# HannesStark/3DInfomax

Hardware: AMD Instinct MI355X
Metric: molecules/sec pretraining step (PNA+Net3D, QM9-50k); PNA-agg HBM GB/s vs peak (higher is better)
Workload: dtype f32

## Files before the change

3dinfomax_amd/csrc/wgrad.hip:

```cpp
#include "common.h"

#include <algorithm>
#include <cstdlib>
#include <cstring>

namespace i3d {
namespace {

typedef float floatx4 __attribute__((ext_vector_type(4)));
typedef int intx4 __attribute__((ext_vector_type(4)));
typedef short shortx4 __attribute__((ext_vector_type(4)));
typedef __bf16 bf16x4_t __attribute__((ext_vector_type(4)));

constexpr int PREC_F32 = 0, PREC_BF16 = 1, PREC_BF16X3 = 2;

__device__ __forceinline__ void split4(const float v[4], shortx4& hi, shortx4& lo, const bool want_lo) {
    const bf16x4_t h = {(__bf16)v[0], (__bf16)v[1], (__bf16)v[2], (__bf16)v[3]};
    hi = __builtin_bit_cast(shortx4, h);
    if (want_lo) {
        const bf16x4_t l = {(__bf16)(v[0] - (float)h[0]), (__bf16)(v[1] - (float)h[1]), (__bf16)(v[2] - (float)h[2]),
                            (__bf16)(v[3] - (float)h[3])};
        lo = __builtin_bit_cast(shortx4, l);
    }
}
typedef __attribute__((address_space(3))) void* lds_ptr_t;

constexpr int WG_T = 13;
constexpr int WG_LD = 208;
constexpr int WG_LDP = 256;
constexpr int WG_BK = 16;
constexpr int wg_nst(int prec) { return prec == 0 ? 2 : 3; }
constexpr int WG_UNIT_FLOATS = WG_T * WG_T * 256;
constexpr int WG_MAX_PROBLEMS = 40;
constexpr int WG_MAX_SLICE = 1024;
constexpr int WG_MAX_OUTPUTS = 8;

struct WgProb {
    const float* A;
    const float* B;
    const int* rows;
    unsigned a_bytes, b_bytes;
    int lda, ldb;
    int M, N;
    int mcw, ncw;
    int m_chunks, n_chunks;
    int k_begin, k_end, k_per_slice;
    int unit_begin;
};

struct WgArgs {
    float* slab;
    unsigned long long* stamps;
    int n_problems, n_units;
    WgProb p[WG_MAX_PROBLEMS];
};

__device__ __forceinline__ int xcd_unit(int total) {
    const int id = blockIdx.x;
    const int q = total / 8, r = total % 8, xcd = id % 8;
    return xcd * q + min(xcd, r) + id / 8;
}

#ifdef WG_TIMING
#define WG_STAMP(i) do { if (threadIdx.x == 0) stamps[i] = __builtin_readcyclecounter(); } while (0)
#else
#define WG_STAMP(i) do { } while (0)
#endif

template <int MT, bool NFULL, int PREC>
__device__ __forceinline__ void wgrad_unit(const WgProb& p, const int slice, const int mc, const int nc, float* __restrict__ out,
                                           float* __restrict__ smem, int* __restrict__ kidx, unsigned long long* stamps) {
    WG_STAMP(0);
    constexpr int NQ = MT == WG_T ? 4 : (MT + 3) / 4;
    const int lane = threadIdx.x & 63, wave = __builtin_amdgcn_readfirstlane(threadIdx.x >> 6);
    const int l15 = lane & 15, lk = lane >> 4;
    const int k0 = p.k_begin + slice * p.k_per_slice;
// ... 17 lines not shown
    float* const Bs = smem + NST * WG_BK * WG_LDP;
    const unsigned as_base = (unsigned)(unsigned long long)(lds_ptr_t)As, bs_base = (unsigned)(unsigned long long)(lds_ptr_t)Bs;
    __syncthreads();

    int rnext[4];
    auto read_rows = [&](int t) {
#pragma unroll
        for (int i = 0; i < 4; ++i) rnext[i] = kidx[min(t * WG_BK + wave + 4 * i, klen - 1)];
    };
    auto issue_piece = [&](int t, int buf, int i) {
        const int kr = wave + 4 * i;
        const int kl = t * WG_BK + kr;
        const bool live = kl < klen && rnext[i] >= 0;
        const unsigned oa = (live && a_ok) ? (unsigned)rnext[i] * lda4 + col : a_rec;
        const unsigned ob = (live && b_ok) ? (unsigned)rnext[i] * ldb4 + col : b_rec;
        const unsigned la = as_base + (unsigned)((buf * WG_BK + kr) * WG_LDP) * 4u;
        const unsigned lb = bs_base + (unsigned)((buf * WG_BK + kr) * WG_LDP) * 4u;
        unsigned keep;
        asm volatile("s_mov_b32 %0, m0\n\ts_mov_b32 m0, %1\n\ts_nop 0\n\tbuffer_load_dwordx4 %2, %3, 0 offen lds\n\t"
                     "s_mov_b32 m0, %4\n\ts_nop 0\n\tbuffer_load_dwordx4 %5, %6, 0 offen lds\n\ts_mov_b32 m0, %0"
                     : "=&s"(keep)
                     : "s"(__builtin_amdgcn_readfirstlane(la)), "v"(oa), "s"(da), "s"(__builtin_amdgcn_readfirstlane(lb)), "v"(ob), "s"(db)
                     : "memory");
    };

    floatx4 acc[3][MT], accx[NQ];
#pragma unroll
    for (int j = 0; j < 3; ++j)
#pragma unroll
        for (int i = 0; i < MT; ++i) acc[j][i] = floatx4{0.f, 0.f, 0.f, 0.f};
#pragma unroll
    for (int q = 0; q < NQ; ++q) accx[q] = floatx4{0.f, 0.f, 0.f, 0.f};

    const int nkt = (klen + WG_BK - 1) / WG_BK;
#pragma unroll
    for (int t0 = 0; t0 < NST - 1; ++t0) {
        read_rows(t0);
#pragma unroll
        for (int i = 0; i < 4; ++i) issue_piece(t0, t0, i);
    }
    if constexpr (NST == 2) asm volatile("s_waitcnt vmcnt(0)" ::: "memory");
    else asm volatile("s_waitcnt vmcnt(8)" ::: "memory");
    __syncthreads();
    WG_STAMP(1);
    const bool extra = ntl == WG_T;
    const int b = lk & 1;
    const int even_off = lk * WG_LDP + l15 + 16 * b, odd_off = lk * WG_LDP + l15 - 16 * b;
    const int own_off = pw ? odd_off : even_off;
    for (int t = 0; t < nkt; ++t) {
        const int cur = t % NST, nxt = (t + NST - 1) % NST;
        read_rows(t + NST - 1);
        const float* as = As + cur * WG_BK * WG_LDP;
        const float* bs = Bs + cur * WG_BK * WG_LDP;
        if constexpr (PREC != PREC_F32) {
            constexpr bool X3 = PREC == PREC_BF16X3;
            auto frag = [&](const float* base, int off, shortx4& hi, shortx4& lo) {
                float v[4];
#pragma unroll
                for (int kk = 0; kk < 4; ++kk) v[kk] = base[kk * 4 * WG_LDP + off];
                split4(v, hi, lo, X3);
            };
            auto fma3 = [&](floatx4& c, const shortx4& bh, const shortx4& bl, const shortx4& ah, const shortx4& al) {
                if constexpr (X3) {
                    c = __builtin_amdgcn_mfma_f32_16x16x16bf16_1k(bl, ah, c, 0, 0, 0);
                    c = __builtin_amdgcn_mfma_f32_16x16x16bf16_1k(bh, al, c, 0, 0, 0);
                }
                c = __builtin_amdgcn_mfma_f32_16x16x16bf16_1k(bh, ah, c, 0, 0, 0);
            };
            shortx4 bh[3], bl[3], bxh, bxl;
#pragma unroll
            for (int j = 0; j < 3; ++j) frag(bs, own_off + (wave + 4 * j) * 16, bh[j], bl[j]);
            frag(bs, even_off + 12 * 16, bxh, bxl);
            constexpr int H0 = (MT + 1) / 2;
#pragma unroll
            for (int half = 0; half < 2; ++half) {
                const int i0 = half ? H0 : 0, cnt = half ? MT - H0 : H0;
                shortx4 ah[H0], al[H0];
#pragma unroll
                for (int i = 0; i < H0; ++i)
                    if (i < cnt) frag(as, (((i0 + i) & 1) ? odd_off : even_off) + (i0 + i) * 16, ah[i], al[i]);
#pragma unroll
                for (int j = 0; j < 3; ++j) {
                    if (NFULL || wave + 4 * j < min(ntl, 12)) {
#pragma unroll
                        for (int i = 0; i < H0; ++i)
                            if (i < cnt) fma3(acc[j][i0 + i], bh[j], bl[j], ah[i], al[i]);
                    }
                    if (j < 2) {
                        __builtin_amdgcn_sched_barrier(0);
                        issue_piece(t + NST - 1, nxt, half * 2 + j);
                        __builtin_amdgcn_sched_barrier(0);
                    }
                }
            }
            if (NFULL || extra) {
#pragma unroll
                for (int q = 0; q < NQ; ++q) {
                    shortx4 xh, xl;
                    if (MT == WG_T && q == 3) frag(as, even_off + 12 * 16, xh, xl);
                    else frag(as, own_off + (wave + 4 * q) * 16, xh, xl);
                    fma3(accx[q], bxh, bxl, xh, xl);
                }
            }
        } else
#pragma unroll
        for (int kk = 0; kk < WG_BK / 4; ++kk) {
            const float* ae = as + kk * 4 * WG_LDP + even_off;
// ... 271 lines not shown
    const long max_units = (workspace_bytes - (1 << 16)) / ((long)WG_UNIT_FLOATS * 4);
#else
    const long max_units = workspace_bytes / ((long)WG_UNIT_FLOATS * 4);
#endif
    static const int fixed_rows = env_int("I3D_WGRAD_ROWS", 0) / WG_BK * WG_BK;
    static const int target_units = env_int("I3D_WGRAD_UNITS", 256);
    int kps;
    if (fixed_rows > 0) {
        kps = std::min(WG_MAX_SLICE, fixed_rows);
        while (kps < WG_MAX_SLICE && plan_units(problems, n_problems, kps) > max_units) kps = std::min(WG_MAX_SLICE, kps * 2);
    } else {
        const long target = std::min<long>(max_units, target_units);
        int lo = 128 / WG_BK, hi = WG_MAX_SLICE / WG_BK;
        while (lo < hi) {
            const int mid = (lo + hi) / 2;
            if (plan_units(problems, n_problems, mid * WG_BK) <= target) hi = mid;
            else lo = mid + 1;
        }
        kps = lo * WG_BK;
    }
    I3D_CHECK_ARG(plan_units(problems, n_problems, kps) <= max_units, "scratch too small");
    WgArgs a;
    WgReduceArgs r;
    a.slab = (float*)workspace;
    a.stamps = nullptr;
#ifdef WG_TIMING
    a.stamps = (unsigned long long*)((char*)workspace + workspace_bytes - (1 << 16));
#endif
    a.n_problems = n_problems;
    int units = 0;
    for (int i = 0; i < n_problems; ++i) {
        const I3dWgradProblem& s = problems[i];
        WgProb& p = a.p[i];
        p.A = s.A; p.B = s.B; p.rows = s.rows;
        p.a_bytes = (unsigned)(((s.rows_total - 1) * s.lda + s.M) * 4);
        p.b_bytes = (unsigned)(((s.rows_total - 1) * s.ldb + s.N) * 4);
        p.lda = s.lda; p.ldb = s.ldb; p.M = s.M; p.N = s.N;
        p.mcw = chunk_width(s.M, p.m_chunks);
        p.ncw = chunk_width(s.N, p.n_chunks);
        p.k_begin = s.k_begin; p.k_end = s.k_begin + s.k_count;
        const int n_slices = cdiv(s.k_count, problem_kps(s, kps));
        p.k_per_slice = n_slices > 0 ? cdiv(cdiv(s.k_count, n_slices), WG_BK) * WG_BK : WG_BK;
        p.unit_begin = units;
        r.unit_begin[i] = units;
        r.n_slices[i] = s.k_count > 0 ? cdiv(s.k_count, p.k_per_slice) : 0;
        units += p.m_chunks * p.n_chunks * r.n_slices[i];
    }
    I3D_CHECK_ARG(units <= max_units, "scratch too small");
    a.n_units = units;
    hipStream_t st = (hipStream_t)stream;
    if (units > 0) {
        const char* const sb = getenv("I3D_WGRAD_SPLIT_BF16");
        const bool split_bf16 = sb != nullptr && sb[0] == '1';
        const int prec = i3d_get_matmul_precision() != 0 ? PREC_BF16 : (split_bf16 ? PREC_BF16X3 : PREC_F32);
        if (prec == PREC_BF16) hipLaunchKernelGGL(wgrad_multi_kernel<PREC_BF16>, dim3(units), dim3(256), 0, st, a);
        else if (prec == PREC_BF16X3) hipLaunchKernelGGL(wgrad_multi_kernel<PREC_BF16X3>, dim3(units), dim3(256), 0, st, a);
        else hipLaunchKernelGGL(wgrad_multi_kernel<PREC_F32>, dim3(units), dim3(256), 0, st, a);
        I3D_CHECK_LAUNCH();
    }
    r.slab = a.slab;
    r.n_outputs = n_outputs;
    long items = 0;
    std::memset(r.coef, 0, sizeof(r.coef));
    for (int i = 0; i < n_outputs; ++i) {
        const I3dWgradOutput& s = outputs[i];
        const WgProb& p = a.p[s.first_problem];
        WgOut& o = r.o[i];
        o.kind = s.kind; o.n_groups = s.n_groups; o.first_problem = s.first_problem;
        o.M = p.M; o.N = p.N; o.mcw = p.mcw; o.ncw = p.ncw; o.m_chunks = p.m_chunks; o.n_chunks = p.n_chunks;
        for (int g = 1; g < s.n_groups; ++g)
            I3D_CHECK_ARG(a.p[s.first_problem + g].M == p.M && a.p[s.first_problem + g].N == p.N, "groups of one output differ in shape");
        o.ldc = s.ldc; o.c_split = s.c_split > 0 ? s.c_split : 0x7fffffff; o.c_delta = s.c_delta;
        o.n_scalers = s.n_scalers; o.scaler_stride = s.scaler_stride;
        o.C = s.C; o.aff = s.aff; o.row = s.row;
        o.item_begin = items;
        items += (long)p.m_chunks * p.n_chunks * WG_T * WG_T * 64;
        if (s.kind == I3D_WGRAD_COMBINE)
            for (int g = 0; g < s.n_groups; ++g)
                for (int k = 0; k < s.n_scalers; ++k) r.coef[g][k] = s.coef[g * s.n_scalers + k];
    }
    r.total_items = items;
    hipLaunchKernelGGL(wgrad_reduce_kernel, dim3(cdiv(items, 256)), dim3(256), 0, st, r);
    I3D_CHECK_LAUNCH();
    return I3D_OK;
}
```

3dinfomax_amd/csrc/panel.hip:

```cpp
#include <stdlib.h>

#include <algorithm>
#include <type_traits>

#include "common.h"

namespace i3d {
namespace {

typedef __bf16 bf16x8 __attribute__((ext_vector_type(8)));
typedef __bf16 bf16x2_t __attribute__((ext_vector_type(2)));
typedef float f32x2_t __attribute__((ext_vector_type(2)));
typedef float floatx4 __attribute__((ext_vector_type(4)));
typedef __attribute__((address_space(3))) void* lds_ptr_t;

constexpr int PN = 208, PT = 13, PBK = 32, PBM = 64;
constexpr int PIECE = 1024;
constexpr int STEP_BYTES = PT * 3 * PIECE;

__device__ __forceinline__ void split_pair(float a, float b, unsigned& hi, unsigned& mid, unsigned& lo) {
    auto pack = [](f32x2_t v) { return __builtin_bit_cast(unsigned, __builtin_convertvector(v, bf16x2_t)); };
    auto widen = [](unsigned u) { f32x2_t r; r.x = __uint_as_float(u << 16); r.y = __uint_as_float(u & 0xffff0000u); return r; };
    f32x2_t v;
    v.x = a; v.y = b;
// ... 208 lines not shown
        float4 b4 = make_float4(0.f, 0.f, 0.f, 0.f);
        if (cok && g.bias != nullptr) b4 = *reinterpret_cast<const float4*>(g.bias + col);
        floatx4 v[RT];
#pragma unroll
        for (int i = 0; i < RT; ++i) {
            v[i] = acc[i][jj];
            v[i][0] += b4.x; v[i][1] += b4.y; v[i][2] += b4.z; v[i][3] += b4.w;
            if (rok[i] && cok) {
                float4* c = reinterpret_cast<float4*>(g.C + (long)(row_lo + 16 * i) * g.ldc + col);
                if (g.accumulate) {
                    const float4 o = *c;
                    v[i][0] += o.x; v[i][1] += o.y; v[i][2] += o.z; v[i][3] += o.w;
                }
                if (STATS) {
#pragma unroll
                    for (int q = 0; q < 4; ++q) v[i][q] = apply_act_c<false>(v[i][q], g.act);
                }
                *c = make_float4(v[i][0], v[i][1], v[i][2], v[i][3]);
            }
        }
        if (STATS) {
            float s[4] = {0.f, 0.f, 0.f, 0.f};
#pragma unroll
            for (int i = 0; i < RT; ++i) {
#pragma unroll
                for (int q = 0; q < 4; ++q) s[q] += rok[i] ? v[i][q] : 0.f;
            }
#pragma unroll
            for (int q = 0; q < 4; ++q) s[q] = row16_sum(s[q]);
            const int rows_here = min(max(g.M - m0, 0), 16 * RT);
            const float cnt = (float)rows_here, inv_cnt = rows_here > 0 ? 1.f / cnt : 0.f;
            float m2[4];
#pragma unroll
            for (int q = 0; q < 4; ++q) {
                const float mean_t = s[q] * inv_cnt;
                m2[q] = 0.f;
#pragma unroll
                for (int i = 0; i < RT; ++i) {
                    const float d = v[i][q] - mean_t;
                    m2[q] += rok[i] ? d * d : 0.f;
                }
                m2[q] = row16_sum(m2[q]);
            }
            if ((lane & 15) == 0 && cok) {
                float* o = g.stats + (long)(blockIdx.x * 2 + rt) * 3 * g.N + col;
                *reinterpret_cast<float4*>(o) = make_float4(s[0], s[1], s[2], s[3]);
                *reinterpret_cast<float4*>(o + g.N) = make_float4(m2[0], m2[1], m2[2], m2[3]);
                *reinterpret_cast<float4*>(o + 2 * g.N) = make_float4(cnt, cnt, cnt, cnt);
            }
        }
    }
}

}
}

using namespace i3d;

extern "C" long i3d_panel_packed_bytes(int N, int K) {
    return (long)cdiv(N, PN) * cdiv(K, PBK) * STEP_BYTES;
}

extern "C" int i3d_panel_pack_multi(const I3dPanelPack* w, int n, void* stream) {
    I3D_CHECK_ARG(w != nullptr && n >= 1 && n <= PACK_MAX, "1..8 weights per launch");
    PackMulti m = {};
    int kt = 1, nb = 1;
    for (int i = 0; i < n; ++i) {
        I3D_CHECK_ARG(w[i].W != nullptr && w[i].packed != nullptr && w[i].N > 0 && w[i].K > 0 && w[i].ldw >= (w[i].trans ? w[i].K : w[i].N) &&
                          (((uintptr_t)w[i].packed) & 15) == 0, "bad arguments");
        m.a[i] = PackArgs{w[i].W, w[i].ldw, w[i].N, w[i].K, w[i].trans, (unsigned short*)w[i].packed};
        kt = std::max(kt, cdiv(w[i].K, PBK));
        nb = std::max(nb, cdiv(w[i].N, PN));
    }
    hipLaunchKernelGGL(panel_pack_kernel, dim3(kt, nb, n), dim3(256), 0, (hipStream_t)stream, m);
    I3D_CHECK_LAUNCH();
    return I3D_OK;
}

extern "C" int i3d_panel_pack(const float* W, int ldw, int N, int K, int trans, void* packed, void* stream) {
    const I3dPanelPack w{W, ldw, N, K, trans, packed};
    return i3d_panel_pack_multi(&w, 1, stream);
}

static int panel_launch(int M, int N, int K, const float* A, int lda, const void* packed, float* C, int ldc, const float* bias,
                        int accumulate, const float* aff, int act, float* stats, void* stream) {
    I3D_CHECK_ARG(M > 0 && N > 0 && K > 0 && A != nullptr && packed != nullptr && C != nullptr, "bad arguments");
    I3D_CHECK_ARG(K % 8 == 0 && N % 4 == 0 && lda % 4 == 0 && ldc % 4 == 0 && lda >= K && ldc >= N, "K % 8, N % 4, 16-byte rows");
    I3D_CHECK_ARG(((((uintptr_t)A) | ((uintptr_t)C) | ((uintptr_t)packed) | ((uintptr_t)bias) | ((uintptr_t)aff) | ((uintptr_t)stats)) & 15) == 0,
                  "16-byte aligned operands");
    I3D_CHECK_ARG(stats == nullptr || relu_class(act), "epilogue activation: none, ReLU or LeakyReLU");
    PanelArgs g{A, lda, M, K, N, (const unsigned char*)packed, C, ldc, bias, accumulate ? 1 : 0, aff, act, stats};
    static const int force_rt = [] { const char* e = getenv("I3D_PANEL_RT"); return e ? atoi(e) : 0; }();
    const bool rt1 = stats == nullptr && (force_rt ? force_rt == 1 : (long)cdiv(M, PBM) * cdiv(N, PN) < 128);
    const dim3 grid(cdiv(M, rt1 ? 32 : PBM), cdiv(N, PN)), block(256);
    hipStream_t s = (hipStream_t)stream;
    if (aff != nullptr && stats != nullptr) hipLaunchKernelGGL((panel_gemm_kernel<true, true, 2>), grid, block, 0, s, g);
    else if (stats != nullptr) hipLaunchKernelGGL((panel_gemm_kernel<false, true, 2>), grid, block, 0, s, g);
    else if (aff != nullptr) {
        if (rt1) hipLaunchKernelGGL((panel_gemm_kernel<true, false, 1>), grid, block, 0, s, g);
        else hipLaunchKernelGGL((panel_gemm_kernel<true, false, 2>), grid, block, 0, s, g);
    } else {
        if (rt1) hipLaunchKernelGGL((panel_gemm_kernel<false, false, 1>), grid, block, 0, s, g);
        else hipLaunchKernelGGL((panel_gemm_kernel<false, false, 2>), grid, block, 0, s, g);
    }
    I3D_CHECK_LAUNCH();
    return I3D_OK;
}

extern "C" int i3d_panel_gemm(int M, int N, int K, const float* A, int lda, const void* packed, float* C, int ldc, const float* bias,
                              int accumulate, void* stream) {
    return panel_launch(M, N, K, A, lda, packed, C, ldc, bias, accumulate, nullptr, I3D_ACT_NONE, nullptr, stream);
}

extern "C" int i3d_panel_stats_tiles(int M) { return 2 * cdiv(M, PBM); }

extern "C" int i3d_panel_gemm_fused(int M, int N, int K, const float* A, int lda, const void* packed, float* C, int ldc, const float* bias,
                                    const float* a_aff, int epi_act, float* stats, void* stream) {
    I3D_CHECK_ARG(stats == nullptr || ((long)N * 4) % 16 == 0, "N % 4");
    return panel_launch(M, N, K, A, lda, packed, C, ldc, bias, 0, a_aff, epi_act, stats, stream);
}
```

3dinfomax_amd/ops.py:

```python
import ctypes
import os
import threading

import torch

from . import _lib
from ._lib import ACT, AGG, SCALER, check, int_array, ptr_array

_tls = threading.local()
KERNEL_TIMERS = None


_raw_stream = torch._C._cuda_getCurrentRawStream


def _stream():
    return _raw_stream(torch.cuda.current_device())


def _p(t):
    return t.data_ptr() if t is not None else None


def _chk(t, dtype=torch.float32):
# ... 536 lines not shown

def bn_finalize_partials(partial, n_tiles, feat, eps, momentum, gamma=None, beta=None, running_mean=None, running_var=None,
                         num_batches_tracked=None, want_aff=True):
    _chk(partial)
    dev = partial.device
    mean = torch.empty(feat, dtype=torch.float32, device=dev)
    invstd = torch.empty(feat, dtype=torch.float32, device=dev)
    aff = torch.empty(3, feat, dtype=torch.float32, device=dev) if want_aff else None
    check(_lib.load().i3d_bn_finalize_partials(_p(partial), n_tiles, feat, float(eps), float(momentum), _p(gamma), _p(beta),
                                               _p(mean), _p(invstd), _p(running_mean), _p(running_var),
                                               _p(num_batches_tracked), _p(aff), _stream()), 'i3d_bn_finalize_partials')
    return mean, invstd, aff


def edge_combine_act_stats(P, Q, bias, src_s, dst_s, act=None, q_code=None):
    _chk(P)
    E, feat = src_s.shape[0], P.shape[1] // 2
    L = _lib.load()
    rpt = L.i3d_edge_stats_rows_per_tile(feat)
    n_tiles = (E + rpt - 1) // rpt
    x = torch.empty(E, feat, dtype=torch.float32, device=P.device)
    partial = torch.empty(n_tiles, 3, feat, dtype=torch.float32, device=P.device)
    check(L.i3d_edge_combine_act_stats(_p(P), P.shape[1], _p(Q), _p(q_code), _p(bias), _p(src_s), _p(dst_s), E, feat, ACT[act],
                                       _p(x), _p(partial), _stream()), 'i3d_edge_combine_act_stats')
    return x, partial, n_tiles


def gemm_fused(A, W, bias=None, a_aff=None, act=None, want_stats=True, out=None, accumulate=False, m_rows=None,
               tile_group=None):
    _chk(A)
    K = A.shape[1]
    if m_rows is not None:
        M, N, stride, rows_total = m_rows.shape[0], W.shape[1], W.shape[1] * W.shape[2], A.shape[0]
    else:
        M, N, stride, rows_total = A.shape[0], W.shape[0], 0, A.shape[0]
    if out is None:
        assert not accumulate
        out = torch.empty(rows_total, N, dtype=torch.float32, device=A.device)
    tiles = (M + 63) // 64
    partial = torch.empty(tiles, 3, N, dtype=torch.float32, device=A.device) if want_stats else None
    check(_lib.load().i3d_gemm_f32_fused(M, N, K, _p(A), K, rows_total, _p(W), K, _p(out), N, _p(bias), int(accumulate),
                                         _p(a_aff), ACT[act], _p(partial), _p(m_rows), _p(tile_group), stride, _stream()),
          'i3d_gemm_f32_fused')
    return out, partial, tiles


def panel_pack(W, trans):
    _chk(W)
    N, K = (W.shape[0], W.shape[1]) if trans else (W.shape[1], W.shape[0])
    L = _lib.load()
    packed = torch.empty(L.i3d_panel_packed_bytes(N, K), dtype=torch.uint8, device=W.device)
    check(L.i3d_panel_pack(_p(W), W.stride(0), N, K, int(bool(trans)), _p(packed), _stream()), 'i3d_panel_pack')
    return packed, N, K


def panel_gemm(A, packed, N, bias=None, out=None, accumulate=False):
    _chk(A)
    M, K = A.shape
    if out is None:
        assert not accumulate
        out = torch.empty(M, N, dtype=torch.float32, device=A.device)
    check(_lib.load().i3d_panel_gemm(M, N, K, _p(A), A.stride(0), _p(packed), _p(out), out.stride(0), _p(bias), int(accumulate), _stream()),
          'i3d_panel_gemm')
    return out


def panel_gemm_fused(A, packed, N, bias=None, a_aff=None, act=None, want_stats=True):
    _chk(A)
    M, K = A.shape
    L = _lib.load()
    out = torch.empty(M, N, dtype=torch.float32, device=A.device)
    tiles = L.i3d_panel_stats_tiles(M)
    partial = torch.empty(tiles, 3, N, dtype=torch.float32, device=A.device) if want_stats else None
    check(L.i3d_panel_gemm_fused(M, N, K, _p(A), A.stride(0), _p(packed), _p(out), N, _p(bias), _p(a_aff), ACT[act], _p(partial), _stream()),
          'i3d_panel_gemm_fused')
    return out, partial, tiles


def gemm_wgrad_bn(dY, x, grad_bias, aff):
    _chk(dY), _chk(x)
    dW = torch.empty(dY.shape[1], x.shape[1], dtype=torch.float32, device=x.device)
    check(_lib.load().i3d_gemm_f32_wgrad_bn(dY.shape[1], x.shape[1], x.shape[0], _p(dY), dY.shape[1], _p(x), x.shape[1], _p(dW),
                                            x.shape[1], _p(grad_bias), _p(aff), _p(_gemm_workspace(x.device)),
                                            GEMM_WORKSPACE_BYTES, _stream()), 'i3d_gemm_f32_wgrad_bn')
    return dW


def pna_aggregate_fwd_aff(e, aff, in_ptr, num_nodes, aggregators, scalers, avg_d_log, force_scalers=False):
    if e.dtype == torch.bfloat16:
        n_s = len(scalers) if (len(scalers) > 1 or force_scalers) else 1
        out = torch.empty(num_nodes, n_s * len(aggregators) * e.shape[1], dtype=torch.float32, device=e.device)
        check(_lib.load().i3d_pna_aggregate_fwd_ex(e.data_ptr(), 1, _p(aff), _p(in_ptr), num_nodes, e.shape[1], int_array(aggregators),
                                                   len(aggregators), int_array(scalers), len(scalers), int(force_scalers),
                                                   float(avg_d_log), _p(out), _stream()), 'i3d_pna_aggregate_fwd_ex')
        return out
    _chk(e)
    n_s = len(scalers) if (len(scalers) > 1 or force_scalers) else 1
    out = torch.empty(num_nodes, n_s * len(aggregators) * e.shape[1], dtype=torch.float32, device=e.device)
    check(_lib.load().i3d_pna_aggregate_fwd_aff(_p(e), _p(aff), _p(in_ptr), num_nodes, e.shape[1], int_array(aggregators),
                                                len(aggregators), int_array(scalers), len(scalers), int(force_scalers),
                                                float(avg_d_log), _p(out), _stream()), 'i3d_pna_aggregate_fwd_aff')
    return out


def pna_aggregate_bwd_aff(grad_out, e, aff, in_ptr, num_nodes, aggregators, scalers, avg_d_log, force_scalers=False):
    if e.dtype == torch.bfloat16:
# ... 789 lines not shown
```

include/infomax3d_hip.h:

```cpp
#ifndef INFOMAX3D_HIP_H
#define INFOMAX3D_HIP_H

#include <stdint.h>

#ifdef __cplusplus
extern "C" {
#endif

#define I3D_OK 0
#define I3D_ERR_INVALID (-1)
#define I3D_ERR_LAUNCH (-2)
#define I3D_NOT_TAKEN 1

#define I3D_ACT_NONE 0
#define I3D_ACT_RELU 1
#define I3D_ACT_SILU 2
#define I3D_ACT_SIGMOID 3
#define I3D_ACT_LEAKY_RELU 4
#define I3D_ACT_TANH 5
#define I3D_ACT_ELU 6
#define I3D_ACT_SELU 7
#define I3D_ACT_SOFTPLUS 8

#define I3D_AGG_MEAN 0
#define I3D_AGG_SUM 1
#define I3D_AGG_MAX 2
#define I3D_AGG_MIN 3
#define I3D_AGG_STD 4
#define I3D_AGG_VAR 5

#define I3D_SCALE_IDENTITY 0
#define I3D_SCALE_AMPLIFICATION 1
#define I3D_SCALE_ATTENUATION 2

int i3d_abi_version(void);
const char* i3d_last_error(void);

int i3d_embedding_sum_fwd(const int64_t* idx, const int* row_perm, int rows, int n_cols, const float* const* tables,
                          int feat, float* out, void* stream);
int i3d_embedding_sum_bwd(const int64_t* idx, const int* row_perm, int rows, int n_cols, const float* grad_out,
                          int feat, float* const* grad_tables, const int* dims, void* stream);

int i3d_pna_aggregate_fwd(const float* e, const int* in_ptr, int num_nodes, int feat, const int* aggregators,
                          int n_aggregators, const int* scalers, int n_scalers, int force_scalers, float avg_d_log,
                          float* out, void* stream);
int i3d_pna_aggregate_bwd(const float* grad_out, const float* e, const int* in_ptr, int num_nodes, int feat,
                          const int* aggregators, int n_aggregators, const int* scalers, int n_scalers,
                          int force_scalers, float avg_d_log, float* grad_e, void* stream);

int i3d_segment_readout_fwd(const float* x, const int* graph_ptr, int num_graphs, int feat, const int* ops,
                            int n_ops, float* out, void* stream);
int i3d_segment_readout_bwd(const float* grad_out, const float* x, const int* graph_ptr, int num_graphs, int feat,
                            const int* ops, int n_ops, float* grad_x, void* stream);

int i3d_gemm_f32(int trans_a, int trans_b, int M, int N, int K, const float* A, int lda, const float* B, int ldb,
                 float* C, int ldc, const float* bias, int accumulate, void* stream);
int i3d_gemm_f32_ex(int trans_a, int trans_b, int M, int N, int K, const float* A, int lda, const float* B, int ldb,
                    float* C, int ldc, const float* bias, int accumulate, int tile_cfg, int splits, void* workspace,
                    long workspace_bytes, void* stream);
int i3d_set_matmul_precision(int bf16);
int i3d_get_matmul_precision(void);
int i3d_set_fp32_products(int split);
int i3d_get_fp32_products(void);

long i3d_panel_packed_bytes(int N, int K);
int i3d_panel_pack(const float* W, int ldw, int N, int K, int trans, void* packed, void* stream);
typedef struct {
    const float* W;
    int ldw, N, K, trans;
    void* packed;
} I3dPanelPack;
int i3d_panel_pack_multi(const I3dPanelPack* weights, int n, void* stream);
int i3d_panel_gemm(int M, int N, int K, const float* A, int lda, const void* packed, float* C, int ldc, const float* bias,
                   int accumulate, void* stream);
int i3d_panel_stats_tiles(int M);
int i3d_panel_gemm_fused(int M, int N, int K, const float* A, int lda, const void* packed, float* C, int ldc, const float* bias,
                         const float* a_aff, int epi_act, float* stats, void* stream);

int i3d_gemm_f32_ws(int trans_a, int trans_b, int M, int N, int K, const float* A, int lda, const float* B, int ldb,
                    float* C, int ldc, const float* bias, int accumulate, void* workspace, long workspace_bytes,
                    void* stream);

int i3d_gemm_f32_blocks(int trans_a, int trans_b, int M, int N, int K, const float* A, int lda, const float* B, int ldb,
                        int b_split, long b_delta, long b_view_floats, float* C, int ldc, int c_split, long c_delta,
                        int accumulate, void* workspace, long workspace_bytes, void* stream);

int i3d_pna_aggregate_fwd_towers(const float* e, const int* in_ptr, int num_nodes, int feat, int tower_feat,
                                 const int* aggregators, int n_aggregators, const int* scalers, int n_scalers,
                                 int force_scalers, float avg_d_log, float* out, void* stream);
int i3d_pna_aggregate_bwd_towers(const float* grad_out, const float* e, const int* in_ptr, int num_nodes, int feat,
                                 int tower_feat, const int* aggregators, int n_aggregators, const int* scalers,
                                 int n_scalers, int force_scalers, float avg_d_log, float* grad_e, void* stream);
int i3d_gemm_f32_batched(int trans_a, int trans_b, int M, int N, int K, const float* A, int lda, long a_batch, const float* B,
                         int ldb, long b_batch, float* C, int ldc, long c_batch, int n_batch, int accumulate, void* workspace,
                         long workspace_bytes, void* stream);

int i3d_gemm_f32_grouped_batched(int trans_b, int m_padded, int N, int K, const float* A, int lda, long a_batch, long a_rows_total,
                                 const int* m_rows, const int* tile_group, const float* B, int ldb, long b_group_stride, long b_batch,
                                 float* C, int ldc, long c_batch, int n_batch, int accumulate, void* stream);

int i3d_pna_combine_weights_fwd(const float* W, int ldw, int f_in, int f_out, int agg_width, int n_groups,
                                int n_scalers, const float* coef, float* WD, void* stream);
int i3d_pna_combine_weights_bwd(const float* dWD, int ldw, int f_in, int f_out, int agg_width, int n_groups,
                                int n_scalers, const float* coef, float* dW, void* stream);
int i3d_gemm_f32_grouped(int trans_b, int m_padded, int N, int K, const float* A, int lda, long a_rows_total,
                         const int* m_rows, const int* tile_group, const float* B, int ldb, long b_group_stride,
                         float* C, int ldc, int accumulate, void* stream);
int i3d_gemm_f32_rowsubset(int M, int N, int n_rows, const float* A, int lda, const float* B, int ldb,
                           const int* k_rows, long rows_total, float* C, int ldc, int accumulate, void* stream);
int i3d_gemm_f32_rowsubset_multi(int M, int N, int n_groups, const int* group_start, const int* group_count,
                                 const float* A, int lda, const float* B, int ldb, const int* k_rows, long rows_total,
                                 float* C, long c_group_stride, int ldc, int accumulate, int tile_cfg, int seg_rows,
                                 void* workspace, long workspace_bytes, void* stream);

long i3d_colreduce_workspace_bytes(int rows, int feat);
int i3d_act_stats_fwd(const float* pre, int rows, int feat, int act, float* x, float eps, float momentum,
                      float* mean, float* invstd, float* running_mean, float* running_var, double* sums_out,
                      void* workspace, void* stream);
int i3d_act_stats_fwd_counted(const float* pre, int rows, int feat, int act, float* x, float eps, float momentum,
                      float* mean, float* invstd, float* running_mean, float* running_var, double* sums_out, long long* num_batches_tracked,
                      void* workspace, void* stream);
int i3d_bn_finalize_stats(const double* sums, int feat, float eps, float momentum, float* mean, float* invstd,
                          float* running_mean, float* running_var, void* stream);
int i3d_bn_apply_fwd(const float* x, int rows, int feat, const float* mean, const float* invstd,
                     const float* gamma, const float* beta, int post_act, const float* residual, float* y,
                     void* stream);
int i3d_bn_eval_fwd(const float* x, int rows, int feat, const float* running_mean, const float* running_var,
                    float eps, const float* gamma, const float* beta, int post_act, const float* residual, float* y,
                    void* stream);
int i3d_bn_bwd(const float* grad_y, const float* x, const float* pre, int rows, int feat, int act, int post_act,
// ... 725 lines not shown
```

Before: 272,900.

## Add split-6 bf16 MFMA weight-gradient path for fp32-exact products

```diff
diff --git a/3dinfomax_amd/csrc/wgrad.hip b/3dinfomax_amd/csrc/wgrad.hip
--- a/3dinfomax_amd/csrc/wgrad.hip
+++ b/3dinfomax_amd/csrc/wgrad.hip
@@ -3,6 +3,7 @@
 #include <algorithm>
 #include <cstdlib>
 #include <cstring>
+#include <type_traits>
 
 namespace i3d {
 namespace {
@@ -11,8 +12,11 @@
 typedef int intx4 __attribute__((ext_vector_type(4)));
 typedef short shortx4 __attribute__((ext_vector_type(4)));
 typedef __bf16 bf16x4_t __attribute__((ext_vector_type(4)));
-
-constexpr int PREC_F32 = 0, PREC_BF16 = 1, PREC_BF16X3 = 2;
+typedef __bf16 bf16x8_t __attribute__((ext_vector_type(8)));
+typedef __bf16 bf16x2_t __attribute__((ext_vector_type(2)));
+typedef float f32x2_t __attribute__((ext_vector_type(2)));
+
+constexpr int PREC_F32 = 0, PREC_BF16 = 1, PREC_BF16X3 = 2, PREC_SPLIT6 = 3;
 
 __device__ __forceinline__ void split4(const float v[4], shortx4& hi, shortx4& lo, const bool want_lo) {
     const bf16x4_t h = {(__bf16)v[0], (__bf16)v[1], (__bf16)v[2], (__bf16)v[3]};
@@ -22,6 +26,32 @@
                             (__bf16)(v[3] - (float)h[3])};
         lo = __builtin_bit_cast(shortx4, l);
     }
+}
+__device__ __forceinline__ void split_pair(float a, float b, unsigned& hi, unsigned& mid, unsigned& lo) {
+    auto pack = [](f32x2_t v) { return __builtin_bit_cast(unsigned, __builtin_convertvector(v, bf16x2_t)); };
+    auto widen = [](unsigned u) { f32x2_t r; r.x = __uint_as_float(u << 16); r.y = __uint_as_float(u & 0xffff0000u); return r; };
+    f32x2_t v;
+    v.x = a; v.y = b;
+    hi = pack(v);
+    const f32x2_t r1 = v - widen(hi);
+    mid = pack(r1);
+    const f32x2_t r2 = r1 - widen(mid);
+    lo = pack(r2);
+}
+typedef unsigned uintx8 __attribute__((ext_vector_type(8)));
+template <bool IS_B>
+__device__ __forceinline__ uintx8 split_windows(const float v[4]) {
+    unsigned hx, hy, mx, my, lx, ly;
+    split_pair(v[0], v[1], hx, mx, lx);
+    split_pair(v[2], v[3], hy, my, ly);
+    if constexpr (IS_B) return uintx8{hx, hy, mx, my, hx, hy, lx, ly};
+    else return uintx8{lx, ly, mx, my, hx, hy, hx, hy};
+}
+template <int STEP>
+__device__ __forceinline__ floatx4 split6_mfma(const uintx8& b, const uintx8& a, const floatx4 c) {
+    constexpr int WA = 2 * STEP, WB = STEP == 0 ? 0 : (STEP == 1 ? 4 : 2);
+    const uint4 aw = {a[WA], a[WA + 1], a[WA + 2], a[WA + 3]}, bw = {b[WB], b[WB + 1], b[WB + 2], b[WB + 3]};
+    return __builtin_amdgcn_mfma_f32_16x16x32_bf16(__builtin_bit_cast(bf16x8_t, bw), __builtin_bit_cast(bf16x8_t, aw), c, 0, 0, 0);
 }
 typedef __attribute__((address_space(3))) void* lds_ptr_t;
 
@@ -145,7 +175,65 @@
         read_rows(t + NST - 1);
         const float* as = As + cur * WG_BK * WG_LDP;
         const float* bs = Bs + cur * WG_BK * WG_LDP;
-        if constexpr (PREC != PREC_F32) {
+        if constexpr (PREC == PREC_SPLIT6) {
+            auto frag_a = [&](const float* base, int off) {
+                float v[4];
+#pragma unroll
+                for (int kk = 0; kk < 4; ++kk) v[kk] = base[kk * 4 * WG_LDP + off];
+                return split_windows<false>(v);
+            };
+            auto frag_b = [&](const float* base, int off) {
+                float v[4];
+#pragma unroll
+                for (int kk = 0; kk < 4; ++kk) v[kk] = base[kk * 4 * WG_LDP + off];
+                return split_windows<true>(v);
+            };
+            uintx8 bf[3], bx;
+#pragma unroll
+            for (int j = 0; j < 3; ++j) bf[j] = frag_b(bs, own_off + (wave + 4 * j) * 16);
+            bx = frag_b(bs, even_off + 12 * 16);
+            const int nt12 = min(ntl, 12);
+            constexpr int H0 = (MT + 1) / 2;
+#pragma unroll
+            for (int half = 0; half < 2; ++half) {
+                const int i0 = half ? H0 : 0, cnt = half ? MT - H0 : H0;
+                uintx8 af[H0];
+#pragma unroll
+                for (int i = 0; i < H0; ++i)
+                    if (i < cnt) af[i] = frag_a(as, (((i0 + i) & 1) ? odd_off : even_off) + (i0 + i) * 16);
+                auto group = [&](auto step) {
+#pragma unroll
+                    for (int j = 0; j < 3; ++j) {
+                        if (NFULL || wave + 4 * j < nt12) {
+#pragma unroll
+                            for (int i = 0; i < H0; ++i)
+                                if (i < cnt) acc[j][i0 + i] = split6_mfma<decltype(step)::value>(bf[j], af[i], acc[j][i0 + i]);
+                        }
+                    }
+                };
+                group(std::integral_constant<int, 0>{});
+                __builtin_amdgcn_sched_barrier(0);
+                issue_piece(t + NST - 1, nxt, half * 2);
+                __builtin_amdgcn_sched_barrier(0);
+                group(std::integral_constant<int, 1>{});
+                __builtin_amdgcn_sched_barrier(0);
+                issue_piece(t + NST - 1, nxt, half * 2 + 1);
+                __builtin_amdgcn_sched_barrier(0);
+                group(std::integral_constant<int, 2>{});
+            }
+            if (NFULL || extra) {
+                uintx8 xf[NQ];
+#pragma unroll
+                for (int q = 0; q < NQ; ++q)
+                    xf[q] = (MT == WG_T && q == 3) ? frag_a(as, even_off + 12 * 16) : frag_a(as, own_off + (wave + 4 * q) * 16);
+#pragma unroll
+                for (int q = 0; q < NQ; ++q) accx[q] = split6_mfma<0>(bx, xf[q], accx[q]);
+#pragma unroll
+                for (int q = 0; q < NQ; ++q) accx[q] = split6_mfma<1>(bx, xf[q], accx[q]);
+#pragma unroll
+                for (int q = 0; q < NQ; ++q) accx[q] = split6_mfma<2>(bx, xf[q], accx[q]);
+            }
+        } else if constexpr (PREC != PREC_F32) {
             constexpr bool X3 = PREC == PREC_BF16X3;
             auto frag = [&](const float* base, int off, shortx4& hi, shortx4& lo) {
                 float v[4];
@@ -523,8 +611,10 @@
     if (units > 0) {
         const char* const sb = getenv("I3D_WGRAD_SPLIT_BF16");
         const bool split_bf16 = sb != nullptr && sb[0] == '1';
-        const int prec = i3d_get_matmul_precision() != 0 ? PREC_BF16 : (split_bf16 ? PREC_BF16X3 : PREC_F32);
+        const int prec = i3d_get_matmul_precision() != 0 ? PREC_BF16
+                         : (split_bf16 ? PREC_BF16X3 : (i3d_get_fp32_products() != 0 ? PREC_SPLIT6 : PREC_F32));
         if (prec == PREC_BF16) hipLaunchKernelGGL(wgrad_multi_kernel<PREC_BF16>, dim3(units), dim3(256), 0, st, a);
+        else if (prec == PREC_SPLIT6) hipLaunchKernelGGL(wgrad_multi_kernel<PREC_SPLIT6>, dim3(units), dim3(256), 0, st, a);
         else if (prec == PREC_BF16X3) hipLaunchKernelGGL(wgrad_multi_kernel<PREC_BF16X3>, dim3(units), dim3(256), 0, st, a);
         else hipLaunchKernelGGL(wgrad_multi_kernel<PREC_F32>, dim3(units), dim3(256), 0, st, a);
         I3D_CHECK_LAUNCH();
```

Result: faster. 278,800, median of 6 (+2.2%).

## Add 8-wave panel GEMM kernel splitting N columns across wave pairs

Applied to the files above, without the earlier changes.

```diff
diff --git a/3dinfomax_amd/csrc/panel.hip b/3dinfomax_amd/csrc/panel.hip
--- a/3dinfomax_amd/csrc/panel.hip
+++ b/3dinfomax_amd/csrc/panel.hip
@@ -284,6 +284,193 @@
     }
 }
 
+template <bool AFF, bool STATS, int CG>
+__global__ void __launch_bounds__(512, 2) panel_gemm8_kernel(PanelArgs g) {
+    I3D_CHAIN_PRIO();
+    static_assert(CG == 2 || (CG == 4 && !STATS), "the statistics tiles are 32 rows: two 16-row waves of a group");
+    __shared__ __attribute__((aligned(16))) unsigned char Bs[2][STEP_BYTES];
+    constexpr int NJ = CG == 2 ? 7 : 4;
+    const int lane = threadIdx.x & 63, wave = __builtin_amdgcn_readfirstlane(threadIdx.x >> 6);
+    const int group = wave >> 2, w4 = wave & 3;
+    const int rt = CG == 2 ? w4 >> 1 : 0, ch = CG == 2 ? (w4 & 1) : w4;
+    const int j0 = CG == 2 ? ch * 7 : (ch ? 1 + 3 * ch : 0), nj = CG == 2 ? (ch ? PT - 7 : 7) : (ch ? 3 : 4);
+    const int cb = blockIdx.y;
+    const int m0 = blockIdx.x * (CG == 2 ? 64 : 32) + group * (CG == 2 ? 32 : 16) + rt * 16;
+    const int KT = (g.K + PBK - 1) / PBK;
+    const unsigned char* bsrc = g.Bp + (long)cb * KT * STEP_BYTES;
+
+    const unsigned bs_base = (unsigned)(unsigned long long)(lds_ptr_t)&Bs[0][0];
+    auto stage_b = [&](int t, int buf) {
+        const unsigned char* src = bsrc + (long)t * STEP_BYTES + lane * 16;
+#pragma unroll
+        for (int i = 0; i < 5; ++i) {
+            const int p = wave + 8 * i;
+            if (p < PT * 3) {
+                unsigned keep;
+                const unsigned dst = __builtin_amdgcn_readfirstlane(bs_base + (unsigned)(buf * STEP_BYTES + p * PIECE));
+                asm volatile("s_mov_b32 %0, m0\n\ts_mov_b32 m0, %2\n\ts_nop 0\n\tglobal_load_lds_dwordx4 %1, off\n\ts_mov_b32 m0, %0"
+                             : "=&s"(keep)
+                             : "v"(src + p * PIECE), "s"(dst)
+                             : "memory");
+            }
+        }
+    };
+    const int arow = lane & 15, akc = (lane >> 4) * 8;
+    const bool arow_ok = m0 + arow < g.M;
+    struct AStep {
+        float4 v[2];
+        float4 f[3][2];
+    };
+    auto load_a = [&](int t, AStep& r) {
+        const int k = t * PBK + akc;
+        if (arow_ok && k < g.K) {
+            const float4* p = reinterpret_cast<const float4*>(g.A + (long)(m0 + arow) * g.lda + k);
+            r.v[0] = p[0];
+            r.v[1] = p[1];
+        } else {
+            r.v[0] = r.v[1] = make_float4(0.f, 0.f, 0.f, 0.f);
+        }
+        if (AFF) {
+            const int kc = min(k, g.K - 8);
+#pragma unroll
+            for (int q = 0; q < 3; ++q) {
+                const float4* p = reinterpret_cast<const float4*>(g.aff + (long)q * g.K + kc);
+                r.f[q][0] = p[0];
+                r.f[q][1] = p[1];
+            }
+        }
+    };
+    auto split_a = [&](int t, const AStep& r, bf16x8& h, bf16x8& m, bf16x8& l) {
+        float4 x0 = r.v[0], x1 = r.v[1];
+        if (AFF) {
+            const bool ok = t * PBK + akc < g.K && arow_ok;
+            auto af = [&](float x, float mu, float sc, float sh) { return ok ? (x - mu) * sc + sh : 0.f; };
+            x0 = make_float4(af(x0.x, r.f[0][0].x, r.f[1][0].x, r.f[2][0].x), af(x0.y, r.f[0][0].y, r.f[1][0].y, r.f[2][0].y),
+                             af(x0.z, r.f[0][0].z, r.f[1][0].z, r.f[2][0].z), af(x0.w, r.f[0][0].w, r.f[1][0].w, r.f[2][0].w));
+            x1 = make_float4(af(x1.x, r.f[0][1].x, r.f[1][1].x, r.f[2][1].x), af(x1.y, r.f[0][1].y, r.f[1][1].y, r.f[2][1].y),
+                             af(x1.z, r.f[0][1].z, r.f[1][1].z, r.f[2][1].z), af(x1.w, r.f[0][1].w, r.f[1][1].w, r.f[2][1].w));
+        }
+        split8(x0, x1, h, m, l);
+    };
+
+    floatx4 acc[NJ];
+#pragma unroll
+    for (int j = 0; j < NJ; ++j) acc[j] = floatx4{0.f, 0.f, 0.f, 0.f};
+
+    bf16x8 ah, am, al;
+    AStep an;
+    stage_b(0, 0);
+    load_a(0, an);
+    split_a(0, an, ah, am, al);
+    for (int t = 0; t < KT; ++t) {
+        asm volatile("s_waitcnt vmcnt(0)" ::: "memory");
+        __syncthreads();
+        if (t + 1 < KT) {
+            load_a(t + 1, an);
+            stage_b(t + 1, (t + 1) & 1);
+        }
+        const unsigned char* bl = &Bs[t & 1][0] + lane * 16;
+#pragma unroll
+        for (int jj = 0; jj < NJ; ++jj) {
+            if (jj < nj) {
+                const int j = j0 + jj;
+                const bf16x8 bh = *reinterpret_cast<const bf16x8*>(bl + (j * 3 + 0) * PIECE);
+                const bf16x8 bm = *reinterpret_cast<const bf16x8*>(bl + (j * 3 + 1) * PIECE);
+                const bf16x8 bo = *reinterpret_cast<const bf16x8*>(bl + (j * 3 + 2) * PIECE);
+                acc[jj] = __builtin_amdgcn_mfma_f32_16x16x32_bf16(bo, ah, acc[jj], 0, 0, 0);
+                acc[jj] = __builtin_amdgcn_mfma_f32_16x16x32_bf16(bh, al, acc[jj], 0, 0, 0);
+                acc[jj] = __builtin_amdgcn_mfma_f32_16x16x32_bf16(bm, am, acc[jj], 0, 0, 0);
+                acc[jj] = __builtin_amdgcn_mfma_f32_16x16x32_bf16(bm, ah, acc[jj], 0, 0, 0);
+                acc[jj] = __builtin_amdgcn_mfma_f32_16x16x32_bf16(bh, am, acc[jj], 0, 0, 0);
+                acc[jj] = __builtin_amdgcn_mfma_f32_16x16x32_bf16(bh, ah, acc[jj], 0, 0, 0);
+            }
+        }
+        __builtin_amdgcn_sched_barrier(0);
+        if (t + 1 < KT) split_a(t + 1, an, ah, am, al);
+    }
+    const int row = m0 + (lane & 15);
+    const bool rok = row < g.M;
+    floatx4 vs[NJ];
+    float4 b4[NJ], o4[NJ];
+#pragma unroll
+    for (int jj = 0; jj < NJ; ++jj) {
+        b4[jj] = o4[jj] = make_float4(0.f, 0.f, 0.f, 0.f);
+        if (jj >= nj) continue;
+        const int col = cb * PN + (j0 + jj) * 16 + (lane >> 4) * 4;
+        const bool cok = col < g.N;
+        if (cok && g.bias != nullptr) b4[jj] = *reinterpret_cast<const float4*>(g.bias + col);
+        if (rok && cok && g.accumulate) o4[jj] = *reinterpret_cast<const float4*>(g.C + (long)row * g.ldc + col);
+    }
+#pragma unroll
+    for (int jj = 0; jj < NJ; ++jj) {
+        floatx4 v = acc[jj];
+        v[0] += b4[jj].x; v[1] += b4[jj].y; v[2] += b4[jj].z; v[3] += b4[jj].w;
+        if (g.accumulate) {
+            v[0] += o4[jj].x; v[1] += o4[jj].y; v[2] += o4[jj].z; v[3] += o4[jj].w;
+        }
+        if (STATS) {
+#pragma unroll
+            for (int q = 0; q < 4; ++q) v[q] = apply_act_c<false>(v[q], g.act);
+        }
+        asm volatile("" : "+v"(v));
+        vs[jj] = v;
+    }
+#pragma unroll
+    for (int jj = 0; jj < NJ; ++jj) {
+        if (jj >= nj) continue;
+        const int col = cb * PN + (j0 + jj) * 16 + (lane >> 4) * 4;
+        if (rok && col < g.N) *reinterpret_cast<float4*>(g.C + (long)row * g.ldc + col) = make_float4(vs[jj][0], vs[jj][1], vs[jj][2], vs[jj][3]);
+    }
+    if (STATS) {
+        float4* xch = reinterpret_cast<float4*>(&Bs[KT & 1][0]) + (group * 2 + ch) * (7 * 64) + lane;
+        if (rt == 1) {
+#pragma unroll
+            for (int jj = 0; jj < NJ; ++jj)
+                if (jj < nj) xch[jj * 64] = make_float4(vs[jj][0], vs[jj][1], vs[jj][2], vs[jj][3]);
+        }
+        __syncthreads();
+        if (rt == 0) {
+            const bool rk[2] = {rok, row + 16 < g.M};
+            const int rows_here = min(max(g.M - m0, 0), 32);
+            const float cnt = (float)rows_here, inv_cnt = rows_here > 0 ? 1.f / cnt : 0.f;
+#pragma unroll
+            for (int jj = 0; jj < NJ; ++jj) {
+                if (jj >= nj) continue;
+                const int col = cb * PN + (j0 + jj) * 16 + (lane >> 4) * 4;
+                const bool cok = col < g.N;
+                const float4 p4 = xch[jj * 64];
+                const floatx4 v[2] = {vs[jj], floatx4{p4.x, p4.y, p4.z, p4.w}};
+                float s[4] = {0.f, 0.f, 0.f, 0.f};
+#pragma unroll
+                for (int i = 0; i < 2; ++i) {
+#pragma unroll
+                    for (int q = 0; q < 4; ++q) s[q] += rk[i] ? v[i][q] : 0.f;
+                }
+#pragma unroll
+                for (int q = 0; q < 4; ++q) s[q] = row16_sum(s[q]);
+                float m2[4];
+#pragma unroll
+                for (int q = 0; q < 4; ++q) {
+                    const float mean_t = s[q] * inv_cnt;
+                    m2[q] = 0.f;
+#pragma unroll
+                    for (int i = 0; i < 2; ++i) {
+                        const float d = v[i][q] - mean_t;
+                        m2[q] += rk[i] ? d * d : 0.f;
+                    }
+                    m2[q] = row16_sum(m2[q]);
+                }
+                if ((lane & 15) == 0 && cok) {
+                    float* o = g.stats + (long)(blockIdx.x * 2 + group) * 3 * g.N + col;
+                    *reinterpret_cast<float4*>(o) = make_float4(s[0], s[1], s[2], s[3]);
+                    *reinterpret_cast<float4*>(o + g.N) = make_float4(m2[0], m2[1], m2[2], m2[3]);
+                    *reinterpret_cast<float4*>(o + 2 * g.N) = make_float4(cnt, cnt, cnt, cnt);
+                }
+            }
+        }
+    }
+}
+
 }
 }
 
@@ -314,6 +501,31 @@
     return i3d_panel_pack_multi(&w, 1, stream);
 }
 
+static int g_panel_form = 0;
+
+extern "C" int i3d_set_panel_form(int form) {
+    if (form != 0 && form != 4 && form != 8 && form != 32) {
+        set_error("%s: invalid argument: %s", __func__, "0: automatic, 4: 4-wave forms, 8: 8-wave form, 32: 8-wave form on 32-row slabs");
+        return I3D_ERR_INVALID;
+    }
+    const int prev = g_panel_form;
+    g_panel_form = form;
+    return prev;
+}
+
+static void launch8(const PanelArgs& g, bool cg4, hipStream_t s) {
+    const dim3 grid(cdiv(g.M, cg4 ? 32 : PBM), cdiv(g.N, PN)), block(512);
+    if (g.aff != nullptr && g.stats != nullptr) hipLaunchKernelGGL((panel_gemm8_kernel<true, true, 2>), grid, block, 0, s, g);
+    else if (g.stats != nullptr) hipLaunchKernelGGL((panel_gemm8_kernel<false, true, 2>), grid, block, 0, s, g);
+    else if (g.aff != nullptr) {
+        if (cg4) hipLaunchKernelGGL((panel_gemm8_kernel<true, false, 4>), grid, block, 0, s, g);
+        else hipLaunchKernelGGL((panel_gemm8_kernel<true, false, 2>), grid, block, 0, s, g);
+    } else {
+        if (cg4) hipLaunchKernelGGL((panel_gemm8_kernel<false, false, 4>), grid, block, 0, s, g);
+        else hipLaunchKernelGGL((panel_gemm8_kernel<false, false, 2>), grid, block, 0, s, g);
+    }
+}
+
 static int panel_launch(int M, int N, int K, const float* A, int lda, const void* packed, float* C, int ldc, const float* bias,
                         int accumulate, const float* aff, int act, float* stats, void* stream) {
     I3D_CHECK_ARG(M > 0 && N > 0 && K > 0 && A != nullptr && packed != nullptr && C != nullptr, "bad arguments");
@@ -322,10 +534,16 @@
                   "16-byte aligned operands");
     I3D_CHECK_ARG(stats == nullptr || relu_class(act), "epilogue activation: none, ReLU or LeakyReLU");
     PanelArgs g{A, lda, M, K, N, (const unsigned char*)packed, C, ldc, bias, accumulate ? 1 : 0, aff, act, stats};
-    static const int force_rt = [] { const char* e = getenv("I3D_PANEL_RT"); return e ? atoi(e) : 0; }();
-    const bool rt1 = stats == nullptr && (force_rt ? force_rt == 1 : (long)cdiv(M, PBM) * cdiv(N, PN) < 128);
+    hipStream_t s = (hipStream_t)stream;
+    const long slabs = (long)cdiv(M, PBM) * cdiv(N, PN);
+    const int form = g_panel_form;
+    if (form == 8 || form == 32 || (form == 0 && aff == nullptr && stats == nullptr)) {
+        launch8(g, stats == nullptr && (form == 32 || (form == 0 && slabs < 128)), s);
+        I3D_CHECK_LAUNCH();
+        return I3D_OK;
+    }
+    const bool rt1 = stats == nullptr && slabs < 128;
     const dim3 grid(cdiv(M, rt1 ? 32 : PBM), cdiv(N, PN)), block(256);
-    hipStream_t s = (hipStream_t)stream;
     if (aff != nullptr && stats != nullptr) hipLaunchKernelGGL((panel_gemm_kernel<true, true, 2>), grid, block, 0, s, g);
     else if (stats != nullptr) hipLaunchKernelGGL((panel_gemm_kernel<false, true, 2>), grid, block, 0, s, g);
     else if (aff != nullptr) {
diff --git a/3dinfomax_amd/ops.py b/3dinfomax_amd/ops.py
--- a/3dinfomax_amd/ops.py
+++ b/3dinfomax_amd/ops.py
@@ -612,6 +612,12 @@
     packed = torch.empty(L.i3d_panel_packed_bytes(N, K), dtype=torch.uint8, device=W.device)
     check(L.i3d_panel_pack(_p(W), W.stride(0), N, K, int(bool(trans)), _p(packed), _stream()), 'i3d_panel_pack')
     return packed, N, K
+
+
+def set_panel_form(form):
+    prev = _lib.load().i3d_set_panel_form(int(form))
+    check(min(prev, 0), 'i3d_set_panel_form')
+    return prev
 
 
 def panel_gemm(A, packed, N, bias=None, out=None, accumulate=False):
diff --git a/include/infomax3d_hip.h b/include/infomax3d_hip.h
--- a/include/infomax3d_hip.h
+++ b/include/infomax3d_hip.h
@@ -76,6 +76,7 @@
 int i3d_panel_stats_tiles(int M);
 int i3d_panel_gemm_fused(int M, int N, int K, const float* A, int lda, const void* packed, float* C, int ldc, const float* bias,
                          const float* a_aff, int epi_act, float* stats, void* stream);
+int i3d_set_panel_form(int form);
 
 int i3d_gemm_f32_ws(int trans_a, int trans_b, int M, int N, int K, const float* A, int lda, const float* B, int ldb,
                     float* C, int ldc, const float* bias, int accumulate, void* workspace, long workspace_bytes,
```

Result: no change. 267,700 before, 265,900 after (-0.6%).
